# leggedrobotics/art_planner

Hardware: NVIDIA H100
Metric: pose-validity checks/s (higher is better)
Workload: dtype f32

## Files before the change

### art_planner_b200/csrc/artp_capi.cu

```cuda
#include <cassert>
#include <climits>
#include <cmath>
#include <cstdlib>
#include <cstring>
#include <cudaTypedefs.h>
#include <type_traits>
#include <vector>

#include "artp_internal.h"
#include "artp_kernels.cuh"
#include "artp_tiles.cuh"

namespace artp_api {

constexpr int kMaxSlices = 9;
constexpr int kMaxStoreSmem = 200 * 1024, kMaxTileSmem = 200 * 1024, kMaxGroupsSmem = 160 * 1024;

struct QueueCtr { uint32_t end, claim; };
struct alignas(32) BoxQueues { QueueCtr big, reach, group; };
struct Counters { BoxQueues q; uint32_t defer; };

struct Shape { int grid = 0, block = 0, smem = 0; };

struct Pipeline {
  enum { kBig, kReach, kGroup };
  Counters* d_ctr = nullptr;
  artp::BoxRec* recs[3] = {};
  uint32_t* d_defer = nullptr;
  size_t recs_cap = 0;
  BoxQueues* d_slices = nullptr;
  unsigned long long* d_compact_state = nullptr;
  size_t compact_state_cap = 0;
  uint32_t compact_epoch = 0;
  artp::TileCfg tile_cfg[2] = {};
  CUtensorMap tile_map[2][2];
  Shape tile[2];
  Shape groups;
  Shape grouping;
  int tcap = 0;
  int tcap_override = 0;
  int mode = 0;
  uint8_t* h_small_out = nullptr;
  bool deferred_unread = false;
  cudaStream_t streams[4] = {};
  cudaStream_t& copy_stream = streams[0];
  cudaStream_t& box_stream = streams[1];
  cudaStream_t& group_stream = streams[2];
  cudaStream_t& tile_stream = streams[3];
  cudaEvent_t order_ev[2 * kMaxSlices + 3] = {};
  cudaEvent_t *const copy_ev = order_ev, *const slice_ev = order_ev + kMaxSlices;
  cudaEvent_t& box_ev = order_ev[2 * kMaxSlices];
  cudaEvent_t &group_ev = order_ev[2 * kMaxSlices + 1], &tile_ev = order_ev[2 * kMaxSlices + 2];
  int timing = 0;
  cudaEvent_t ev[6] = {};
  bool ev_valid = false;
  ~Pipeline() {
    for (cudaStream_t s : streams) if (s) { cudaStreamSynchronize(s); cudaStreamDestroy(s); }
    for (cudaEvent_t e : order_ev) if (e) cudaEventDestroy(e);
    for (cudaEvent_t e : ev) if (e) cudaEventDestroy(e);
    for (artp::BoxRec* r : recs) cudaFree(r);
    cudaFree(d_ctr); cudaFree(d_defer); cudaFree(d_slices); cudaFree(d_compact_state);
    if (h_small_out) cudaFreeHost(h_small_out);
  }
};

}

using namespace artp_api;

namespace {

thread_local std::string g_create_error;

__global__ void reverse_columns_kernel(const float* __restrict__ layer, float* __restrict__ H, int nx, int nz, int pitch) {
  const size_t total = (size_t)pitch * nz;
  for (size_t i = blockIdx.x * (size_t)blockDim.x + threadIdx.x; i < total; i += (size_t)gridDim.x * blockDim.x) {
    const int z = (int)(i / pitch), x = (int)(i - (size_t)z * pitch);
    H[i] = (x < nx) ? layer[x + (size_t)(nz - 1 - z) * nx] * 1.0f + 0.0f : 0.0f;
  }
}

__global__ void build_level_kernel(const float* __restrict__ H, const float2* __restrict__ prevT,
                                   const unsigned char* __restrict__ prevNF, const unsigned char* __restrict__ mergeable,
                                   float2* __restrict__ T, unsigned char* __restrict__ NF, int nx, int nz, int pitch, int half) {
  const size_t total = (size_t)pitch * nz;
  for (size_t i = blockIdx.x * (size_t)blockDim.x + threadIdx.x; i < total; i += (size_t)gridDim.x * blockDim.x) {
    const int z = (int)(i / pitch), x = (int)(i - (size_t)z * pitch);
    if (x >= nx) { T[i] = make_float2(0.f, 0.f); NF[i] = 0; continue; }
    const int x2 = min(x + half, nx - 1), z2 = min(z + half, nz - 1);
    const size_t id[4] = {(size_t)z * pitch + x, (size_t)z * pitch + x2, (size_t)z2 * pitch + x, (size_t)z2 * pitch + x2};
    float mx = -CUDART_INF_F, mn = CUDART_INF_F;
    unsigned char nf = 0;
#pragma unroll
    for (int q = 0; q < 4; ++q) {
      if (prevT) {
        const float2 v = prevT[id[q]];
        mx = fmaxf(mx, v.x); mn = fminf(mn, v.y); nf |= prevNF[id[q]];
      } else {
        const float h = H[id[q]];
        mx = fmaxf(mx, h);
        if (fabsf(h) < CUDART_INF_F) mn = fminf(mn, h); else nf |= 1;
        nf |= mergeable[id[q]];
      }
    }
    T[i] = make_float2(mx, mn);
    NF[i] = nf;
  }
}

__global__ void build_codes_kernel(const float2* __restrict__ T, const unsigned char* __restrict__ NF, uint32_t* __restrict__ C,
                                   size_t n, float base, float step) {
  const float top = artp::code_dec(base, step, artp::kCodeMax);
  for (size_t i = blockIdx.x * (size_t)blockDim.x + threadIdx.x; i < n; i += (size_t)gridDim.x * blockDim.x) {
    const float2 v = T[i];
    uint32_t cM = 0, cm = artp::kCodeNone;
    if (v.x > top) cM = artp::kCodeNone;
    else if (v.x > -CUDART_INF_F) {
      uint32_t lo = 1, hi = artp::kCodeMax;
      while (lo < hi) {
        const uint32_t mid = (lo + hi) >> 1;
        if (artp::code_dec(base, step, mid) >= v.x) hi = mid; else lo = mid + 1;
      }
      cM = lo;
    }
    if (v.y <= top) {
      uint32_t lo = 0, hi = artp::kCodeMax;
      while (lo < hi) {
        const uint32_t mid = (lo + hi + 1) >> 1;
        if (artp::code_dec(base, step, mid) <= v.y) lo = mid; else hi = mid - 1;
      }
      cm = lo;
    }
    C[i] = artp::code_word(cM, cm, NF[i] & 3u);
  }
}

void code_scale_of(float lo, float hi, float& base, float& step) {
  base = lo <= hi ? lo : 0.0f;
  int e = -126;
  while (e < 127 && artp::code_dec(base, std::ldexp(1.0f, e), artp::kCodeMax) < hi) ++e;
  step = std::ldexp(1.0f, e);
}
void code_scale(const float* layer, size_t n, float& base, float& step) {
  float lo = HUGE_VALF, hi = -HUGE_VALF;
  for (size_t i = 0; i < n; ++i) {
    const float v = layer[i] * 1.0f + 0.0f;
    if (std::fabs(v) < HUGE_VALF) { lo = std::min(lo, v); hi = std::max(hi, v); }
  }
  code_scale_of(lo, hi, base, step);
}

struct PlaneSlot { unsigned long long key; uint32_t lo, hi; };
constexpr unsigned long long kEmptyKey = ~0ull;
__device__ __forceinline__ unsigned long long plane_key(int kx, int kz, int kd) {
  return ((unsigned long long)(uint32_t)(kx & 0xffff) << 48) | ((unsigned long long)(uint32_t)(kz & 0xffff) << 32) | (uint32_t)kd;
}
__device__ __forceinline__ uint32_t plane_slot_hash(unsigned long long k) {
  k ^= k >> 33; k *= 0xff51afd7ed558ccdull; k ^= k >> 33; k *= 0xc4ceb9fe1a85ec53ull; k ^= k >> 33;
  return (uint32_t)k;
}
__global__ void plane_table_clear_kernel(PlaneSlot* tab, size_t cap) {
  for (size_t i = blockIdx.x * (size_t)blockDim.x + threadIdx.x; i < cap; i += (size_t)gridDim.x * blockDim.x) {
    tab[i].key = kEmptyKey; tab[i].lo = 0xffffffffu; tab[i].hi = 0u;
  }
}
__device__ __forceinline__ bool cell_tri_plane(const artp::Field& f, int x, int x_off, int z, int u, float pl[4]) {
  float hA, hB, hC, hD;
  artp::load_cell(f, x, z, hA, hB, hC, hD);
  const bool ok = u == 0 ? (artp::finitef(hA) && artp::finitef(hB) && artp::finitef(hC))
// ... 363 lines not shown
int check_states(Handle* h, const T* d_states, size_t n, uint8_t* d_valid, cudaStream_t s, const HostFeed* feed = nullptr) {
  artp::Work w;
  if constexpr (std::is_same_v<T, float>) w.s2f = d_states; else w.s2 = d_states;
  w.valid = d_valid;
  w.n_items = (uint32_t)n;
  return run_items(h, w, s, feed);
}

template <typename T>
int check_poses(Handle* h, const T* states, size_t n, uint8_t* valid, bool on_device, cudaStream_t stream) {
  TRY(check_common(h, n));
  if (n == 0) return ARTP_OK;
  if (!states || !valid) return null_buffer(h);
  if (on_device) {
    CU_TRY(h, cudaSetDevice(h->device));
    ChainScope cs(h, 0, stream);
    if (cs.rc) return cs.rc;
    return check_states(h, states, n, valid, stream);
  }
  if (n <= (size_t)artp::kSmallBatch && !h->pipe->timing) {
    artp::SmallBatch sb;
    for (size_t i = 0; i < n * 7; ++i) (&sb.s[0][0])[i] = (double)states[i];
    return check_poses_small(h, sb, n, valid);
  }
  char* r[2];
  TRY(host_call_begin(h, {n * 7 * sizeof(T), n}, r));
  const HostFeed feed = std::is_same_v<T, float>
                            ? HostFeed{(const char*)states, r[0], 7 * sizeof(T), 256 * 1024, {0.08f, 0.17f, 0.25f, 0.25f, 0.25f}}
                            : HostFeed{(const char*)states, r[0], 7 * sizeof(T), 128 * 1024, {0.06f, 0.14f, 0.20f, 0.20f, 0.20f, 0.20f}};
  TRY(check_states(h, (const T*)r[0], n, (uint8_t*)r[1], h->stream, &feed));
  CU_TRY(h, cudaMemcpyAsync(valid, r[1], n, cudaMemcpyDeviceToHost, h->stream));
  return host_call_end(h, true);
}

int motion_items(Handle* h, size_t n, int n_steps) {
  if (n_steps < 0) { h->err = "n_steps < 0"; return ARTP_E_INVALID; }
  return check_common(h, n * ((size_t)n_steps + 1));
}
int check_motions_on(Handle* h, const double* d_s1, const double* d_s2, size_t n, int n_steps, uint8_t* d_valid, cudaStream_t s) {
  TRY(launch(h, fill_u8_kernel, grid_for(h, n, 256, 8), 256, 0, s, d_valid, n, 1));
  const size_t items = n * ((size_t)n_steps + 1);
  artp::Work w;
  w.s1 = d_s1; w.s2 = d_s2; w.valid = d_valid; w.n_items = (uint32_t)items; w.steps = n_steps; w.edge_mode = 1;
  return run_items(h, w, s);
}

__global__ void edge_prefix_kernel(const uint8_t* __restrict__ item_valid, const uint32_t* __restrict__ item_off, size_t n,
                                   int32_t* __restrict__ valid_prefix) {
  for (size_t e = blockIdx.x * (size_t)blockDim.x + threadIdx.x; e < n; e += (size_t)gridDim.x * blockDim.x) {
    const uint32_t o0 = item_off[e];
    valid_prefix[e] = (int32_t)artp::leading_valid(item_valid + o0, item_off[e + 1] - o0);
  }
}

int check_items_prefix(Handle* h, const double* d_s1, const double* d_s2, size_t n, const uint32_t* d_item_off,
                       size_t total_items, uint8_t* d_item_valid, int32_t* d_valid_prefix, void* stream, int quotient) {
  TRY(check_common(h, total_items));
  if (n == 0) return ARTP_OK;
  if (!d_s1 || !d_s2 || !d_item_off || !d_valid_prefix || (total_items && !d_item_valid)) {
    return null_buffer(h);
  }
  if (n >= 0xFFFFFFFFull) { h->err = "too many edges"; return ARTP_E_INVALID; }
  CU_TRY(h, cudaSetDevice(h->device));
  cudaStream_t s = (cudaStream_t)stream;
  ChainScope cs(h, 0, s);
  if (cs.rc) return cs.rc;
  if (total_items) {
    artp::Work w;
    w.s1 = d_s1; w.s2 = d_s2; w.valid = d_item_valid; w.n_items = (uint32_t)total_items;
    w.item_off = d_item_off; w.n_edges = (uint32_t)n; w.quotient = quotient;
    TRY(run_items(h, w, s));
  }
  return launch(h, edge_prefix_kernel, grid_for(h, n, 256, 8), 256, 0, s, d_item_valid, d_item_off, n, d_valid_prefix);
}

int check_items_prefix_host(Handle* h, const double* s1, const double* s2, const std::vector<uint32_t>& off, int quotient,
                            int32_t* valid_prefix) {
  const size_t n = off.size() - 1, total = off[n], sb = n * 7 * sizeof(double);
  char* r[5];
  TRY(host_call_begin(h, {sb, sb, (n + 1) * sizeof(uint32_t), n * sizeof(int32_t), total}, r));
  CU_TRY(h, cudaMemcpyAsync(r[0], s1, sb, cudaMemcpyHostToDevice, h->stream));
  CU_TRY(h, cudaMemcpyAsync(r[1], s2, sb, cudaMemcpyHostToDevice, h->stream));
  CU_TRY(h, cudaMemcpyAsync(r[2], off.data(), (n + 1) * sizeof(uint32_t), cudaMemcpyHostToDevice, h->stream));
  TRY(check_items_prefix(h, (const double*)r[0], (const double*)r[1], n, (const uint32_t*)r[2], total, (uint8_t*)r[4],
                         (int32_t*)r[3], h->stream, quotient));
  CU_TRY(h, cudaMemcpyAsync(valid_prefix, r[3], n * sizeof(int32_t), cudaMemcpyDeviceToHost, h->stream));
  return host_call_end(h, true);
}

int pack_valid_bits(Handle* h, const uint8_t* d_valid, size_t n, uint32_t* d_bits, cudaStream_t s) {
  if (n == 0) return ARTP_OK;
  if (!d_valid || !d_bits) return null_buffer(h);
  CU_TRY(h, cudaSetDevice(h->device));
  const size_t words = (n + 31) / 32;
  return launch(h, pack_bits_kernel, grid_for(h, words * 32, 256, 8), 256, 0, s, d_valid, n, d_bits);
}

int timed_round_ms(Handle* h, float* ms, std::initializer_list<std::pair<int, int>> pairs) {
  const Pipeline& p = *h->pipe;
  if (!ms) return ARTP_E_INVALID;
  if (!p.timing || !p.ev_valid) { h->err = "timing not enabled or no call recorded"; return ARTP_E_INVALID; }
  CU_TRY(h, cudaSetDevice(h->device));
  CU_TRY(h, cudaEventSynchronize(p.ev[5]));
  for (const auto& [from, to] : pairs) CU_TRY(h, cudaEventElapsedTime(ms++, p.ev[from], p.ev[to]));
  return ARTP_OK;
}

template <typename... P>
int fit_shape(Handle* h, void (*kernel)(P...), int block, int smem, Shape& out) {
  int per_sm = 0;
  CU_TRY(h, cudaOccupancyMaxActiveBlocksPerMultiprocessor(&per_sm, kernel, block, smem));
  out = {h->sm_count * std::max(per_sm, 1), block, smem};
  return ARTP_OK;
}

int set_shapes(Handle* h, const int span[2][2], int tcap, int store) {
  Pipeline& p = *h->pipe;
  TRY(fit_shape(h, artp::box_items_block_kernel, artp::kBlockStageThreads, store, p.grouping));
  p.tcap = tcap;
  PFN_cuTensorMapEncodeTiled encode = nullptr;
  cudaDriverEntryPointQueryResult qres;
  if (cudaGetDriverEntryPoint("cuTensorMapEncodeTiled", (void**)&encode, cudaEnableDefault, &qres) != cudaSuccess || !encode) {
    h->err = "cuTensorMapEncodeTiled not available from the driver"; return ARTP_E_CUDA;
  }
  h->chk.reach_tw = 0; h->chk.reach_th = 0;
  for (int q = 0; q < 2; ++q) {
    const int tw = std::min((span[q][0] + 3 + 3 + 3) & ~3, 256), th = std::min(span[q][1] + 3, 256);
    artp::TileCfg tc;
    tc.tw = tw; tc.th = th; tc.bytes = (uint32_t)tw * th * 4; tc.stride = (tc.bytes + 127u) & ~127u;
    tc.slots = (tc.stride > 2048) ? 1 : 2;
    int wpc = 8;
    while (wpc > 1 && (size_t)wpc * tc.slots * tc.stride + 128 > 72 * 1024) wpc >>= 1;
    if ((size_t)wpc * tc.slots * tc.stride + 128 > kMaxTileSmem) {
      if (q == 1) { p.tile[1] = Shape{}; continue; }
      tc.tw = 64; tc.th = 64; tc.bytes = 64 * 64 * 4; tc.stride = tc.bytes; tc.slots = 1; wpc = 4;
    }
    const cuuint64_t gdim[2] = {(cuuint64_t)h->pitch, (cuuint64_t)h->cols};
    const cuuint64_t gstr[1] = {(cuuint64_t)h->pitch * sizeof(float)};
    const cuuint32_t box[2] = {(cuuint32_t)tc.tw, (cuuint32_t)tc.th};
    const cuuint32_t one[2] = {1, 1};
    for (int layer = 0; layer < 2; ++layer) {
      const CUresult cr = encode(&p.tile_map[q][layer], CU_TENSOR_MAP_DATA_TYPE_FLOAT32, 2, h->d_H[layer], gdim, gstr, box, one,
                                 CU_TENSOR_MAP_INTERLEAVE_NONE, CU_TENSOR_MAP_SWIZZLE_NONE, CU_TENSOR_MAP_L2_PROMOTION_L2_128B,
                                 CU_TENSOR_MAP_FLOAT_OOB_FILL_NONE);
      if (cr != CUDA_SUCCESS) { h->err = "cuTensorMapEncodeTiled failed (" + std::to_string((int)cr) + ")"; return ARTP_E_CUDA; }
    }
    tc.x_off = h->win_row0;
    p.tile_cfg[q] = tc;
    p.tile[q] = {0, wpc * 32, (int)((size_t)wpc * tc.slots * tc.stride + 128)};
    if (q == 1) { h->chk.reach_tw = tc.tw; h->chk.reach_th = tc.th; }
  }
  p.groups = Shape{};
  if (h->chk.reach_tw && p.tile_cfg[1].tw <= 127 && p.tile_cfg[1].th <= 255) {
    const int gsm = artp::kMaxTileWarps * 8 * (int)p.tile_cfg[1].stride + 128;
    if (gsm <= kMaxGroupsSmem && !std::getenv("ARTP_NO_GROUPS")) {
      TRY(fit_shape(h, artp::reach_groups_kernel, artp::kMaxTileWarps * 32, gsm, p.groups));
    }
  }
  for (Shape& t : p.tile)
    if (t.block) TRY(fit_shape(h, artp::box_tiles_warp_kernel, t.block, t.smem, t));
  return ARTP_OK;
}

}

int artp_api::take_sticky_error(Handle* h) {
  if (h->h_err && *(volatile uint32_t*)h->h_err) {
    const uint32_t e = *(volatile uint32_t*)h->h_err;
    *(volatile uint32_t*)h->h_err = 0;
    if (e & 2u) {
      h->err = "a box reached outside this handle's map window (artp_set_map_window: route samples to the shard that holds them, "
               "halo >= box half-diagonal + offsets); affected poses were marked invalid";
      return ARTP_E_WINDOW;
    }
    h->err = "plane-grouping stage overflow: a zone exceeded its shared-memory store; affected poses were marked invalid";
    return ARTP_E_LIMIT;
  }
  return ARTP_OK;
}

int artp_api::check_states_f32(Handle* h, const float* d_states, size_t n, uint8_t* d_valid, cudaStream_t s) {
  return check_states(h, d_states, n, d_valid, s);
}

int artp_api::check_states_cta(Handle* h, const double* d_states, const uint32_t* d_count, const uint32_t* d_stop, size_t max_n,
                               uint8_t* d_valid, cudaStream_t s) {
  if (max_n == 0) return ARTP_OK;
  TRY(launch(h, artp::pose_states_kernel, (unsigned)max_n, 256, h->pipe->grouping.smem, s, h->chk, d_states, d_count, d_stop,
             d_valid, h->pipe->tcap, h->d_err));
  h->pipe->ev_valid = false;
  return ARTP_OK;
}

int artp_api::compact_valid(Handle* h, const uint8_t* d_valid, size_t n, int64_t base, void* d_indices, uint32_t* d_count,
                            cudaStream_t s, bool bits, bool u32) {
  Pipeline& p = *h->pipe;
  if (n == 0) { CU_TRY(h, cudaMemsetAsync(d_count, 0, sizeof(uint32_t), s)); return ARTP_OK; }
  ChainScope cs(h, 1, s);
  if (cs.rc) return cs.rc;
  const size_t nt = (n + kCompactTile - 1) / kCompactTile;
  if (p.compact_state_cap < nt + 1 || p.compact_epoch + 1 >= kCompactEpochs) {
    TRY(grow(h, p.d_compact_state, p.compact_state_cap, nt + 1));
    CU_TRY(h, cudaMemsetAsync(p.d_compact_state, 0, p.compact_state_cap * sizeof(unsigned long long), s));
    p.compact_epoch = 0;
  }
  const uint32_t epoch = ++p.compact_epoch;
  auto run = [&](auto kernel, auto* indices) {
    return launch(h, kernel, (unsigned)nt, kCompactThreads, 0, s, d_valid, n, base, p.d_compact_state, epoch, indices, d_count);
  };
  if (bits) return run(compact_kernel<true, int64_t>, (int64_t*)d_indices);
  if (u32) return run(compact_kernel<false, uint32_t>, (uint32_t*)d_indices);
  return run(compact_kernel<false, int64_t>, (int64_t*)d_indices);
}

extern "C" {

const char* artp_version(void) { return "artp 0.1 sm_90a"; }

const char* artp_last_error(const artp_handle* hh) {
  if (!hh) return g_create_error.c_str();
  return reinterpret_cast<const Handle*>(hh)->err.c_str();
}

int artp_create(const artp_params* params, artp_handle** out) {
  if (!params || !out) { g_create_error = "null argument"; return ARTP_E_INVALID; }
  *out = nullptr;
  int ndev = 0;
  cudaError_t e = cudaGetDeviceCount(&ndev);
  if (e != cudaSuccess || ndev == 0) {
    g_create_error = std::string("no CUDA device: ") + cudaGetErrorString(e);
    return ARTP_E_CUDA;
  }
  if (params->device < 0 || params->device >= ndev) { g_create_error = "bad device ordinal"; return ARTP_E_INVALID; }
  if (!(params->torso_length > 0 && params->torso_width > 0 && params->torso_height > 0 && params->reach_x > 0 &&
        params->reach_y > 0 && params->reach_z > 0)) {
    g_create_error = "box dimensions must be positive";
    return ARTP_E_INVALID;
  }
  Handle* h = new Handle();
  h->p = *params;
  h->device = params->device;
  auto fail = [&](const char* what, cudaError_t ce) {
    g_create_error = std::string(what) + ": " + cudaGetErrorString(ce);
    artp_destroy(reinterpret_cast<artp_handle*>(h));
    return ARTP_E_CUDA;
  };
  if ((e = cudaSetDevice(h->device)) != cudaSuccess) return fail("cudaSetDevice", e);
  cudaDeviceProp prop;
  if ((e = cudaGetDeviceProperties(&prop, h->device)) != cudaSuccess) return fail("cudaGetDeviceProperties", e);
  h->sm_count = prop.multiProcessorCount;
  cudaFuncAttributes fa;
  if ((e = cudaFuncGetAttributes(&fa, artp::box_tiles_warp_kernel)) != cudaSuccess)
    return fail("no usable kernel image (built for sm_90a)", e);
  int prio_least = 0, prio_greatest = 0;
  if ((e = cudaDeviceGetStreamPriorityRange(&prio_least, &prio_greatest)) != cudaSuccess) return fail("cudaDeviceGetStreamPriorityRange", e);
  if ((e = cudaStreamCreateWithFlags(&h->stream, cudaStreamNonBlocking)) != cudaSuccess) return fail("cudaStreamCreate", e);
  Pipeline& p = *(h->pipe = new Pipeline());
  for (cudaStream_t& st : p.streams) {
    e = &st == &p.tile_stream ? cudaStreamCreateWithPriority(&st, cudaStreamNonBlocking, prio_greatest)
                              : cudaStreamCreateWithFlags(&st, cudaStreamNonBlocking);
    if (e != cudaSuccess) return fail("cudaStreamCreate", e);
  }
  for (cudaEvent_t& ev : p.order_ev)
    if ((e = cudaEventCreateWithFlags(&ev, cudaEventDisableTiming)) != cudaSuccess) return fail("cudaEventCreate", e);
  for (cudaEvent_t& ev : h->chain_ev)
    if ((e = cudaEventCreateWithFlags(&ev, cudaEventDisableTiming)) != cudaSuccess) return fail("cudaEventCreate", e);
  if ((e = cudaMalloc(&p.d_slices, kMaxSlices * sizeof(BoxQueues))) != cudaSuccess) return fail("cudaMalloc", e);
  if ((e = cudaMalloc(&p.d_ctr, sizeof(Counters))) != cudaSuccess) return fail("cudaMalloc", e);
  if ((e = cudaHostAlloc((void**)&p.h_small_out, 64, cudaHostAllocMapped)) != cudaSuccess) return fail("cudaHostAlloc", e);
  const std::pair<const void*, int> smem_caps[] = {
      {(const void*)artp::pose_small_kernel, kMaxStoreSmem}, {(const void*)artp::pose_states_kernel, kMaxStoreSmem},
      {(const void*)artp::box_items_block_kernel, kMaxStoreSmem}, {(const void*)artp::box_tiles_warp_kernel, kMaxTileSmem},
      {(const void*)artp::reach_groups_kernel, kMaxGroupsSmem}};
  for (const auto& [k, bytes] : smem_caps)
    if ((e = cudaFuncSetAttribute(k, cudaFuncAttributeMaxDynamicSharedMemorySize, bytes)) != cudaSuccess)
      return fail("cudaFuncSetAttribute", e);
  if ((e = cudaHostAlloc((void**)&h->h_err, 64, cudaHostAllocMapped)) != cudaSuccess) return fail("cudaHostAlloc", e);
  *h->h_err = 0;
  if ((e = cudaHostGetDevicePointer((void**)&h->d_err, h->h_err, 0)) != cudaSuccess) return fail("cudaHostGetDevicePointer", e);
  h->cnn = artp_cnn::create(h->device, h->sm_count);
  artp::Checker& c = h->chk;
  std::memset(&c, 0, sizeof(c));
  c.side[0][0] = (float)params->torso_length; c.side[0][1] = (float)params->torso_width; c.side[0][2] = (float)params->torso_height;
  c.side[1][0] = (float)params->reach_x; c.side[1][1] = (float)params->reach_y; c.side[1][2] = (float)params->reach_z;
  c.torso_off[0] = (float)params->torso_off_x; c.torso_off[1] = (float)params->torso_off_y;
  c.torso_off[2] = (float)(params->torso_off_z - params->feet_off_z);
  c.feet_ox = (float)params->feet_off_x; c.feet_oy = (float)params->feet_off_y;
  c.unknown_untraversable = params->unknown_space_untraversable ? 1 : 0;
  *out = reinterpret_cast<artp_handle*>(h);
  return ARTP_OK;
}

void artp_destroy(artp_handle* hh) {
  if (!hh) return;
  Handle* h = reinterpret_cast<Handle*>(hh);
  cudaSetDevice(h->device);
  if (h->stream) { cudaStreamSynchronize(h->stream); cudaStreamDestroy(h->stream); }
  delete h->pipe;
  for (int k = 0; k < 2; ++k) for (int l = 0; l <= artp::kMaxLevel; ++l) { cudaFree(h->d_T[k][l]); cudaFree(h->d_C[k][l]); }
  cudaFree(h->d_H[0]); cudaFree(h->d_H[1]); cudaFree(h->d_stage); cudaFree(h->d_simplify);
  sampling_free(h);
  roadmap_free(h);
  planner_free(h);
  if (h->h_err) cudaFreeHost(h->h_err);
  for (cudaEvent_t ev : h->chain_ev) if (ev) cudaEventDestroy(ev);
  artp_cnn::destroy(h->cnn);
  delete h;
// ... 378 lines not shown
```

### art_planner_b200/csrc/artp_tiles.cuh

```cuda
#pragma once

#include <cuda.h>

#include "artp_kernels.cuh"

namespace artp {

constexpr uint32_t kDeferReachBit = 0x80000000u;
constexpr int kTileChunk = 8;

__device__ __forceinline__ uint32_t smem_addr(const void* p) { return (uint32_t)__cvta_generic_to_shared(p); }
__device__ __forceinline__ void mbar_init(uint64_t* bar, uint32_t count) {
  asm volatile("mbarrier.init.shared::cta.b64 [%0], %1;" ::"r"(smem_addr(bar)), "r"(count));
}
__device__ __forceinline__ void mbar_expect_tx(uint64_t* bar, uint32_t bytes) {
  asm volatile("mbarrier.arrive.expect_tx.shared::cta.b64 _, [%0], %1;" ::"r"(smem_addr(bar)), "r"(bytes) : "memory");
}
__device__ __forceinline__ void mbar_wait(uint64_t* bar, uint32_t parity) {
  asm volatile(
      "{\n\t"
      ".reg .pred P1;\n\t"
      "TWAIT_LOOP:\n\t"
      "mbarrier.try_wait.parity.shared::cta.b64 P1, [%0], %1;\n\t"
      "@P1 bra TWAIT_DONE;\n\t"
      "bra TWAIT_LOOP;\n\t"
      "TWAIT_DONE:\n\t"
      "}" ::"r"(smem_addr(bar)), "r"(parity) : "memory");
}
__device__ __forceinline__ void tma_tile_2d(void* dst, const CUtensorMap* map, uint64_t* bar, int c0, int c1) {
  asm volatile(
      "cp.async.bulk.tensor.2d.shared::cluster.global.mbarrier::complete_tx::bytes [%0], [%1, {%3, %4}], [%2];" ::"r"(
          smem_addr(dst)),
      "l"(map), "r"(smem_addr(bar)), "r"(c0), "r"(c1)
      : "memory");
}

constexpr int kMaxTileWarps = 8;

__device__ __forceinline__ unsigned char* warp_tile_slots(unsigned char* smem, const TileCfg& tc, int n, uint64_t bars[2]) {
  const int wid = threadIdx.x >> 5;
  unsigned char* slots = reinterpret_cast<unsigned char*>((reinterpret_cast<uintptr_t>(smem) + 127) & ~(uintptr_t)127) +
                         (size_t)wid * n * tc.stride;
  if ((threadIdx.x & 31) == 0) { mbar_init(&bars[0], 1); mbar_init(&bars[1], 1); }
  asm volatile("fence.mbarrier_init.release.cluster;" ::: "memory");
  __syncwarp();
  return slots;
}

__global__ void __launch_bounds__(kMaxTileWarps * 32, 3)
box_tiles_warp_kernel(const Checker c, const __grid_constant__ CUtensorMap map0, const __grid_constant__ CUtensorMap map1,
                      const TileCfg tc, const Work w, const BoxRec* __restrict__ recs, const uint32_t* __restrict__ rec_count,
                      uint32_t* __restrict__ work_counter, uint32_t* __restrict__ defer_count, uint32_t* __restrict__ defer_list,
                      uint32_t queue_bit, int force_defer) {
  extern __shared__ __align__(128) unsigned char tile_smem[];
  __shared__ WarpScratch ws_all[kMaxTileWarps];
  __shared__ uint64_t bars[kMaxTileWarps][2];
  const int lane = threadIdx.x & 31, wid = threadIdx.x >> 5;
  WarpScratch& ws = ws_all[wid];
  unsigned char* slots = warp_tile_slots(tile_smem, tc, tc.slots, bars[wid]);
  uint32_t phase[2] = {0u, 0u};
  const uint32_t total = *rec_count;
  auto prefetch = [&](uint32_t ri, int slot) {
    const int x0 = rec_x0(recs + ri), z0 = rec_z0(recs + ri);
    const uint32_t fl = rec_flags(recs + ri);
    if (lane == 0) {
      mbar_expect_tx(&bars[wid][slot], tc.bytes);
      tma_tile_2d(slots + (size_t)slot * tc.stride, (fl & 7u) ? &map1 : &map0, &bars[wid][slot], (x0 & ~3) - tc.x_off, z0);
    }
  };
  const uint32_t nwarps2 = 2u * gridDim.x * (blockDim.x >> 5);
  uint32_t next_r0 = 0, next_n = 0;
  const uint32_t first_seen = *(volatile const uint32_t*)work_counter;
  const bool fixed_claims = total - min(first_seen, total) >= (nwarps2 >> 2) * (uint32_t)kTileChunk;
  auto claim = [&]() {
    if (lane == 0) {
      next_n = (uint32_t)kTileChunk;
      if (!fixed_claims) {
        const uint32_t cur = *(volatile const uint32_t*)work_counter;
        next_n = cur < total ? min(max((total - cur) / nwarps2, 1u), (uint32_t)kTileChunk) : 1u;
      }
      next_r0 = atomicAdd(work_counter, next_n);
    }
  };
  if (!fixed_claims) claim();
  for (;;) {
    if (fixed_claims) claim();
    const uint32_t r0 = __shfl_sync(kFull, next_r0, 0), nclaim = __shfl_sync(kFull, next_n, 0);
    if (r0 >= total) break;
    if (!fixed_claims) claim();
    const uint32_t r1 = min(r0 + nclaim, total);
    if (force_defer) {
      if (lane == 0) for (uint32_t ri = r0; ri < r1; ++ri) defer_list[atomicAdd(defer_count, 1u)] = ri | queue_bit;
      continue;
    }
    for (uint32_t ri = r0; ri < r1; ++ri) {
      const int slot = (int)(ri - r0) & (tc.slots - 1);
      if (tc.slots == 1 || ri == r0) { __syncwarp(); prefetch(ri, slot); }
      const BoxRec r = load_rec(recs + ri);
      if (tc.slots == 2 && ri + 1 < r1) { __syncwarp(); prefetch(ri + 1, slot ^ 1); }
      const uint32_t slot_item = r.item;
      const bool foot = (r.flags & 7) != 0;
      int dead = 0;
      if (lane == 0) dead = (*(volatile const uint8_t*)(w.valid + slot_item) == 0);
      dead = __shfl_sync(kFull, dead, 0);
      mbar_wait(&bars[wid][slot], phase[slot]);
      phase[slot] ^= 1u;
      if (dead) continue;
      BoxCtx b;
      rec_to_ctx(c, r, b);
      int res;
      if ((b.x1 - b.x0) + 4 > tc.tw || (b.z1 - b.z0) + 1 > tc.th) {
        res = R_DEFER;
      } else {
        const ZoneView zv{reinterpret_cast<const float*>(slots + (size_t)slot * tc.stride) + (b.x0 & 3), tc.tw};
        res = box_collide_warp<true>(foot ? c.f[1] : c.f[0], b, zv, ws, lane, c.cell_margin, (r.flags & REC_NEEDS_REDUCE) != 0,
                                     (r.flags & REC_ALLFINITE) != 0, (r.flags & REC_MERGEFREE) != 0);
      }
      if (lane == 0) {
        if (res == R_DEFER) defer_list[atomicAdd(defer_count, 1u)] = ri | queue_bit;
        else if (box_fails(foot, res)) w.valid[slot_item] = 0;
      }
    }
  }
}

constexpr int kGroupRounds = 8;
constexpr int kGroupTasks = 64;

__global__ void __launch_bounds__(kMaxTileWarps * 32, 3)
reach_groups_kernel(const Checker c, const __grid_constant__ CUtensorMap map1, const TileCfg tc, const Work w,
                    const BoxRec* __restrict__ recs, const uint32_t* __restrict__ rec_count, uint32_t* __restrict__ work_counter) {
  extern __shared__ __align__(128) unsigned char tile_smem[];
  __shared__ uint64_t bars[kMaxTileWarps][2];
  __shared__ uint16_t tasks_all[kMaxTileWarps][4][kGroupTasks];
  __shared__ __align__(16) float ctx_all[kMaxTileWarps][4][16];
  const int lane = threadIdx.x & 31, wid = threadIdx.x >> 5, g = lane >> 3, gl = lane & 7;
  const Field& f = c.f[1];
  unsigned char* slots = warp_tile_slots(tile_smem, tc, 8, bars[wid]);
  uint16_t* tasks = tasks_all[wid][g];
  uint32_t phase = 0u;
  const uint32_t total = *rec_count;
  const unsigned gshift = (unsigned)g * 8u;
  auto prefetch = [&](uint32_t first, int slot) {
    const uint32_t ri = first + (uint32_t)g;
    int x0 = 0, z0 = 0;
    const bool act = ri < total;
    if (act && gl == 0) { x0 = rec_x0(recs + ri); z0 = rec_z0(recs + ri); }
    const int nact = (int)min(4u, total - first);
    if (lane == 0) mbar_expect_tx(&bars[wid][slot], (uint32_t)nact * tc.bytes);
#pragma unroll 1
    for (int q = 0; q < nact; ++q) {
      const int sx = __shfl_sync(kFull, x0, q * 8), sz = __shfl_sync(kFull, z0, q * 8);
      if (lane == 0) tma_tile_2d(slots + (size_t)(slot * 4 + q) * tc.stride, &map1, &bars[wid][slot], (sx & ~3) - tc.x_off, sz);
    }
  };
  const uint32_t nwarps8 = 8u * gridDim.x * (blockDim.x >> 5);
  uint32_t next_r0 = 0, next_n = 0;
  auto claim = [&]() {
    if (lane == 0) {
      const uint32_t cur = *(volatile const uint32_t*)work_counter;
      next_n = 4u * (cur < total ? min(max((total - cur) / nwarps8, 1u), (uint32_t)kGroupRounds) : 1u);
      next_r0 = atomicAdd(work_counter, next_n);
    }
  };
  claim();
  for (;;) {
    const uint32_t r0 = __shfl_sync(kFull, next_r0, 0), nclaim = __shfl_sync(kFull, next_n, 0);
    if (r0 >= total) break;
    claim();
    const int nrounds = (int)((min(r0 + nclaim, total) - r0 + 3u) / 4u);
    __syncwarp();
    prefetch(r0, 0);
#pragma unroll 1
    for (int round = 0; round < nrounds; ++round) {
      const int slot = round & 1;
      const uint32_t ri = r0 + 4u * (uint32_t)round + (uint32_t)g;
      const bool act = ri < total;
      BoxRec r = {};
      if (act) r = load_rec(recs + ri);
      if (round + 1 < nrounds) { __syncwarp(); prefetch(r0 + 4u * (uint32_t)(round + 1), slot ^ 1); }
      int alive = 0;
      if (act && gl == 0) alive = (*(volatile const uint8_t*)(w.valid + r.item) != 0);
      alive = __shfl_sync(kFull, alive, 0, 8);
      mbar_wait(&bars[wid][slot], (phase >> slot) & 1u);
      phase ^= 1u << slot;
      __syncwarp();
      bool gdone = !(act && alive);
      BoxCtx b;
      rec_to_ctx(c, r, b);
      if (gdone) { b.x0 = b.z0 = 0; b.x1 = b.z1 = 1; }
      if (gl == 0) {
        float* cx = ctx_all[wid][g];
#pragma unroll
        for (int i = 0; i < 9; ++i) cx[i] = b.R1[i];
        cx[9] = b.P[0]; cx[10] = b.P[1]; cx[11] = b.P[2]; cx[12] = b.minB;
        cx[13] = __int_as_float(b.x0); cx[14] = __int_as_float(b.z0);
      }
      const float* tile = reinterpret_cast<const float*>(slots + (size_t)(slot * 4 + g) * tc.stride) + (b.x0 & 3);
      const float top = b.maxB + (1e-4f + 4e-6f * fabsf(b.maxB));
      bool ghit = false;
      const bool allFinite = (r.flags & REC_ALLFINITE) != 0;
      {
        const float xr = box_half_extent(b.R1, b.side, 0) + 1e-4f, zr = box_half_extent(b.R1, b.side, 2) + 1e-4f;
        const int vx0 = max(b.x0, (int)ceilf((b.P[0] - xr) * f.iW)), vx1 = min(b.x1, (int)floorf((b.P[0] + xr) * f.iW));
        const int vz0 = max(b.z0, (int)ceilf((b.P[2] - zr) * f.iD)), vz1 = min(b.z1, (int)floorf((b.P[2] + zr) * f.iD));
        const int nXi = max(vx1 - vx0 + 1, 0), nZi = max(vz1 - vz0 + 1, 0), nVi = nXi * nZi;
        const float* tin = tile + (vz0 - b.z0) * tc.tw + (vx0 - b.x0);
        int maxNV = gdone ? 0 : nVi;
        maxNV = __reduce_max_sync(kFull, maxNV);
        const uint32_t magicX = magic_for(nXi);
#pragma unroll 1
        for (int t0 = 0; t0 < maxNV; t0 += 8) {
          const int t = t0 + gl;
          bool hit = false;
          if (!gdone && t < nVi) {
            const int zi = (nXi > 1) ? (int)__umulhi((uint32_t)t, magicX) : t, xi = t - zi * nXi;
            const float h = tin[zi * tc.tw + xi];
            hit = h > b.minB && h < top && vertex_inside(b, (vx0 + xi) * f.sW, h, (vz0 + zi) * f.sD);
            if (hit && !allFinite)
              hit = vertex_in_kept_triangle<true>(ZoneView{tile, tc.tw}, b.x1 - b.x0 + 1, b.z1 - b.z0 + 1, vx0 - b.x0 + xi,
                                                  vz0 - b.z0 + zi, b.minB);
          }
          if ((__ballot_sync(kFull, hit) >> gshift) & 0xffu) { ghit = true; gdone = true; }
          if (__all_sync(kFull, gdone)) break;
        }
      }
      __syncwarp();
      int nt = 0;
      {
        float pc[3];
        box_corner(b, gl, pc);
        const float gx = pc[0] * f.iW, gz = pc[2] * f.iD;
        const int cxl = (int)floorf(gx - c.cell_margin), cxh = (int)floorf(gx + c.cell_margin);
        const int czl = (int)floorf(gz - c.cell_margin), czh = (int)floorf(gz + c.cell_margin);
        const int oxl = __shfl_xor_sync(kFull, cxl, 4), oxh = __shfl_xor_sync(kFull, cxh, 4);
        const int ozl = __shfl_xor_sync(kFull, czl, 4), ozh = __shfl_xor_sync(kFull, czh, 4);
        const bool same = (oxl == cxl) & (oxh == cxh) & (ozl == czl) & (ozh == czh);
        const bool mine = !gdone && !((gl & 4) && same);
        bool ok[4];
#pragma unroll
        for (int sub = 0; sub < 4; ++sub) {
          const int ccx = (sub & 1) ? cxh : cxl, ccz = (sub & 2) ? czh : czl;
          ok[sub] = mine && !((sub & 1) && cxh == cxl) && !((sub & 2) && czh == czl) && ccx >= b.x0 && ccx < b.x1 && ccz >= b.z0 &&
                    ccz < b.z1;
        }
        int base = 0;
#pragma unroll
        for (int sub = 0; sub < 4; ++sub) {
          const unsigned gm = (__ballot_sync(kFull, ok[sub]) >> gshift) & 0xffu;
          if (ok[sub]) {
            const int slot_i = base + __popc(gm & ((1u << gl) - 1u));
            const int ccx = (sub & 1) ? cxh : cxl, ccz = (sub & 2) ? czh : czl;
            const int code = (((ccx - b.x0) << 8) | (ccz - b.z0)) << 1;
            tasks[2 * slot_i] = (uint16_t)code; tasks[2 * slot_i + 1] = (uint16_t)(code | 1);
          }
          base += __popc(gm);
        }
        nt = 2 * base;
      }
      __syncwarp();
      {
        const int n0 = __shfl_sync(kFull, nt, 0), n1 = __shfl_sync(kFull, nt, 8), n2 = __shfl_sync(kFull, nt, 16), n3 = __shfl_sync(kFull, nt, 24);
        const int o1 = n0, o2 = n0 + n1, o3 = o2 + n2, NT = o3 + n3;
        unsigned hit_groups = 0u;
#pragma unroll 1
        for (int j0 = 0; j0 < NT; j0 += 32) {
          const int j = j0 + lane;
          if (j < NT) {
            const int gi = (j >= o1) + (j >= o2) + (j >= o3);
            const int q = j - (gi == 0 ? 0 : gi == 1 ? o1 : gi == 2 ? o2 : o3);
            const int tk = tasks_all[wid][gi][q];
            const float4* cx = reinterpret_cast<const float4*>(ctx_all[wid][gi]);
            const float4 c0 = cx[0], c1 = cx[1], c2 = cx[2], c3 = cx[3];
            BoxCtx tb;
            tb.R1[0] = c0.x; tb.R1[1] = c0.y; tb.R1[2] = c0.z; tb.R1[3] = c0.w; tb.R1[4] = c1.x; tb.R1[5] = c1.y; tb.R1[6] = c1.z;
            tb.R1[7] = c1.w; tb.R1[8] = c2.x; tb.P[0] = c2.y; tb.P[1] = c2.z; tb.P[2] = c2.w; tb.minB = c3.x;
            tb.side[0] = c.side[1][0]; tb.side[1] = c.side[1][1]; tb.side[2] = c.side[1][2];
            const int tx0 = __float_as_int(c3.y), tz0 = __float_as_int(c3.z);
            const bool isUp = (tk & 1) == 0;
            const int lx = tk >> 9, lz = (tk >> 1) & 0xff, ccx = tx0 + lx, ccz = tz0 + lz;
            const float* p = reinterpret_cast<const float*>(slots + (size_t)(slot * 4 + gi) * tc.stride) + (tx0 & 3) + lz * tc.tw + lx;
            const float hA = p[0], hB = p[1], hC = p[tc.tw], hD = p[tc.tw + 1];
            if (tri_kept(isUp, hA, hB, hC, hD, tb.minB)) {
              float pl[4], cxs[4], czs[4];
              cell_plane(f, isUp, ccx, ccz, hA, hB, hC, hD, pl);
              const int nc = box_plane(tb, pl, 4, cxs, czs);
              const int tcx = isUp ? ccx : ccx + 1, tcz = isUp ? ccz : ccz + 1;
              bool hit = false;
#pragma unroll
              for (int i = 0; i < 4; ++i) hit = hit || (i < nc && on_tri(f, isUp, tcx, tcz, cxs[i], czs[i]));
              if (hit) hit_groups |= 1u << gi;
            }
          }
        }
        __syncwarp();
        hit_groups = __reduce_or_sync(kFull, hit_groups);
        if ((hit_groups >> g) & 1u) ghit = true;
      }
      if (gl == 0 && act && alive && box_fails(true, ghit ? R_HIT : R_FREE)) w.valid[r.item] = 0;
      __syncwarp();
    }
  }
}

}
```

Before: 2.068 billion.

## Compact surviving reach boxes into a ring before the plane stage

Splits the reach-groups kernel into two phases. Boxes that survive the vertex stage are appended to a per-warp ring of up to 8 contexts, and the plane-test stage runs only once four live boxes have accumulated, so warp lanes are not wasted on groups that already finished. Tile slots move from fixed double-buffered pairs to an 11-slot pool tracked by a free bitmask, and the shared-memory cap is raised to fit them. The cost is more shared memory per block, which may reduce occupancy, plus extra bookkeeping. There is also a risk of slot exhaustion or ordering bugs, because the ring holds tiles across rounds.

```diff
diff --git a/art_planner_b200/csrc/artp_capi.cu b/art_planner_b200/csrc/artp_capi.cu
--- a/art_planner_b200/csrc/artp_capi.cu
+++ b/art_planner_b200/csrc/artp_capi.cu
@@ -14,7 +14,7 @@
 namespace artp_api {
 
 constexpr int kMaxSlices = 9;
-constexpr int kMaxStoreSmem = 200 * 1024, kMaxTileSmem = 200 * 1024, kMaxGroupsSmem = 160 * 1024;
+constexpr int kMaxStoreSmem = 200 * 1024, kMaxTileSmem = 200 * 1024, kMaxGroupsSmem = 216 * 1024;
 
 struct QueueCtr { uint32_t end, claim; };
 struct alignas(32) BoxQueues { QueueCtr big, reach, group; };
@@ -684,7 +684,7 @@
   }
   p.groups = Shape{};
   if (h->chk.reach_tw && p.tile_cfg[1].tw <= 127 && p.tile_cfg[1].th <= 255) {
-    const int gsm = artp::kMaxTileWarps * 8 * (int)p.tile_cfg[1].stride + 128;
+    const int gsm = artp::kMaxTileWarps * artp::kGroupSlots * (int)p.tile_cfg[1].stride + 128;
     if (gsm <= kMaxGroupsSmem && !std::getenv("ARTP_NO_GROUPS")) {
       TRY(fit_shape(h, artp::reach_groups_kernel, artp::kMaxTileWarps * 32, gsm, p.groups));
     }
diff --git a/art_planner_b200/csrc/artp_tiles.cuh b/art_planner_b200/csrc/artp_tiles.cuh
--- a/art_planner_b200/csrc/artp_tiles.cuh
+++ b/art_planner_b200/csrc/artp_tiles.cuh
@@ -126,6 +126,8 @@
 
 constexpr int kGroupRounds = 8;
 constexpr int kGroupTasks = 64;
+constexpr int kGroupSlots = 11;
+constexpr int kGroupRing = 8;
 
 __global__ void __launch_bounds__(kMaxTileWarps * 32, 3)
 reach_groups_kernel(const Checker c, const __grid_constant__ CUtensorMap map1, const TileCfg tc, const Work w,
@@ -133,26 +135,34 @@
   extern __shared__ __align__(128) unsigned char tile_smem[];
   __shared__ uint64_t bars[kMaxTileWarps][2];
   __shared__ uint16_t tasks_all[kMaxTileWarps][4][kGroupTasks];
-  __shared__ __align__(16) float ctx_all[kMaxTileWarps][4][16];
+  __shared__ __align__(16) float ring_ctx[kMaxTileWarps][kGroupRing][16];
+  __shared__ uint32_t ring_item[kMaxTileWarps][kGroupRing];
+  __shared__ uint8_t ring_slot[kMaxTileWarps][kGroupRing];
   const int lane = threadIdx.x & 31, wid = threadIdx.x >> 5, g = lane >> 3, gl = lane & 7;
   const Field& f = c.f[1];
-  unsigned char* slots = warp_tile_slots(tile_smem, tc, 8, bars[wid]);
+  unsigned char* slots = warp_tile_slots(tile_smem, tc, kGroupSlots, bars[wid]);
   uint16_t* tasks = tasks_all[wid][g];
   uint32_t phase = 0u;
+  uint32_t free_slots = (1u << kGroupSlots) - 1u;
+  int head = 0, nring = 0;
   const uint32_t total = *rec_count;
   const unsigned gshift = (unsigned)g * 8u;
-  auto prefetch = [&](uint32_t first, int slot) {
+  auto prefetch = [&](uint32_t first, int bar) {
     const uint32_t ri = first + (uint32_t)g;
     int x0 = 0, z0 = 0;
-    const bool act = ri < total;
-    if (act && gl == 0) { x0 = rec_x0(recs + ri); z0 = rec_z0(recs + ri); }
+    if (ri < total && gl == 0) { x0 = rec_x0(recs + ri); z0 = rec_z0(recs + ri); }
     const int nact = (int)min(4u, total - first);
-    if (lane == 0) mbar_expect_tx(&bars[wid][slot], (uint32_t)nact * tc.bytes);
+    if (lane == 0) mbar_expect_tx(&bars[wid][bar], (uint32_t)nact * tc.bytes);
+    int mine = 0;
 #pragma unroll 1
     for (int q = 0; q < nact; ++q) {
+      const int s = __ffs(free_slots) - 1;
+      free_slots &= free_slots - 1u;
+      if (g == q) mine = s;
       const int sx = __shfl_sync(kFull, x0, q * 8), sz = __shfl_sync(kFull, z0, q * 8);
-      if (lane == 0) tma_tile_2d(slots + (size_t)(slot * 4 + q) * tc.stride, &map1, &bars[wid][slot], (sx & ~3) - tc.x_off, sz);
-    }
+      if (lane == 0) tma_tile_2d(slots + (size_t)s * tc.stride, &map1, &bars[wid][bar], (sx & ~3) - tc.x_off, sz);
+    }
+    return mine;
   };
   const uint32_t nwarps8 = 8u * gridDim.x * (blockDim.x >> 5);
   uint32_t next_r0 = 0, next_n = 0;
@@ -164,41 +174,40 @@
     }
   };
   claim();
+  uint32_t r0 = 0;
+  int round = 0, nrounds = 0, next_slot = 0;
+  bool more = true;
   for (;;) {
-    const uint32_t r0 = __shfl_sync(kFull, next_r0, 0), nclaim = __shfl_sync(kFull, next_n, 0);
-    if (r0 >= total) break;
-    claim();
-    const int nrounds = (int)((min(r0 + nclaim, total) - r0 + 3u) / 4u);
-    __syncwarp();
-    prefetch(r0, 0);
-#pragma unroll 1
-    for (int round = 0; round < nrounds; ++round) {
-      const int slot = round & 1;
+    if (round == nrounds && more) {
+      r0 = __shfl_sync(kFull, next_r0, 0);
+      const uint32_t nclaim = __shfl_sync(kFull, next_n, 0);
+      more = r0 < total;
+      if (more) {
+        claim();
+        nrounds = (int)((min(r0 + nclaim, total) - r0 + 3u) / 4u);
+        round = 0;
+        __syncwarp();
+        next_slot = prefetch(r0, 0);
+      }
+    }
+    if (round < nrounds) {
+      const int bar = round & 1, slot = next_slot;
       const uint32_t ri = r0 + 4u * (uint32_t)round + (uint32_t)g;
       const bool act = ri < total;
       BoxRec r = {};
       if (act) r = load_rec(recs + ri);
-      if (round + 1 < nrounds) { __syncwarp(); prefetch(r0 + 4u * (uint32_t)(round + 1), slot ^ 1); }
+      if (round + 1 < nrounds) { __syncwarp(); next_slot = prefetch(r0 + 4u * (uint32_t)(round + 1), bar ^ 1); }
       int alive = 0;
       if (act && gl == 0) alive = (*(volatile const uint8_t*)(w.valid + r.item) != 0);
       alive = __shfl_sync(kFull, alive, 0, 8);
-      mbar_wait(&bars[wid][slot], (phase >> slot) & 1u);
-      phase ^= 1u << slot;
+      mbar_wait(&bars[wid][bar], (phase >> bar) & 1u);
+      phase ^= 1u << bar;
       __syncwarp();
       bool gdone = !(act && alive);
       BoxCtx b;
       rec_to_ctx(c, r, b);
-      if (gdone) { b.x0 = b.z0 = 0; b.x1 = b.z1 = 1; }
-      if (gl == 0) {
-        float* cx = ctx_all[wid][g];
-#pragma unroll
-        for (int i = 0; i < 9; ++i) cx[i] = b.R1[i];
-        cx[9] = b.P[0]; cx[10] = b.P[1]; cx[11] = b.P[2]; cx[12] = b.minB;
-        cx[13] = __int_as_float(b.x0); cx[14] = __int_as_float(b.z0);
-      }
-      const float* tile = reinterpret_cast<const float*>(slots + (size_t)(slot * 4 + g) * tc.stride) + (b.x0 & 3);
+      const float* tile = reinterpret_cast<const float*>(slots + (size_t)slot * tc.stride) + (b.x0 & 3);
       const float top = b.maxB + (1e-4f + 4e-6f * fabsf(b.maxB));
-      bool ghit = false;
       const bool allFinite = (r.flags & REC_ALLFINITE) != 0;
       {
         const float xr = box_half_extent(b.R1, b.side, 0) + 1e-4f, zr = box_half_extent(b.R1, b.side, 2) + 1e-4f;
@@ -221,85 +230,125 @@
               hit = vertex_in_kept_triangle<true>(ZoneView{tile, tc.tw}, b.x1 - b.x0 + 1, b.z1 - b.z0 + 1, vx0 - b.x0 + xi,
                                                   vz0 - b.z0 + zi, b.minB);
           }
-          if ((__ballot_sync(kFull, hit) >> gshift) & 0xffu) { ghit = true; gdone = true; }
+          if ((__ballot_sync(kFull, hit) >> gshift) & 0xffu) gdone = true;
           if (__all_sync(kFull, gdone)) break;
         }
       }
-      __syncwarp();
-      int nt = 0;
-      {
-        float pc[3];
-        box_corner(b, gl, pc);
-        const float gx = pc[0] * f.iW, gz = pc[2] * f.iD;
-        const int cxl = (int)floorf(gx - c.cell_margin), cxh = (int)floorf(gx + c.cell_margin);
-        const int czl = (int)floorf(gz - c.cell_margin), czh = (int)floorf(gz + c.cell_margin);
-        const int oxl = __shfl_xor_sync(kFull, cxl, 4), oxh = __shfl_xor_sync(kFull, cxh, 4);
-        const int ozl = __shfl_xor_sync(kFull, czl, 4), ozh = __shfl_xor_sync(kFull, czh, 4);
-        const bool same = (oxl == cxl) & (oxh == cxh) & (ozl == czl) & (ozh == czh);
-        const bool mine = !gdone && !((gl & 4) && same);
-        bool ok[4];
+      const unsigned surv = __ballot_sync(kFull, !gdone && gl == 0);
+      if (!gdone && gl == 0) {
+        const int e = (head + nring + __popc(surv & ((1u << lane) - 1u))) & (kGroupRing - 1);
+        float4* cx = reinterpret_cast<float4*>(ring_ctx[wid][e]);
+        cx[0] = make_float4(b.R1[0], b.R1[1], b.R1[2], b.R1[3]);
+        cx[1] = make_float4(b.R1[4], b.R1[5], b.R1[6], b.R1[7]);
+        cx[2] = make_float4(b.R1[8], b.P[0], b.P[1], b.P[2]);
+        cx[3] = make_float4(b.minB, __int_as_float(b.x0), __int_as_float(b.z0), __int_as_float((b.x1 - b.x0) | ((b.z1 - b.z0) << 16)));
+        ring_item[wid][e] = r.item;
+        ring_slot[wid][e] = (uint8_t)slot;
+      }
+      free_slots |= __reduce_or_sync(kFull, (act && gdone && gl == 0) ? 1u << slot : 0u);
+      nring += __popc(surv);
+      ++round;
+    }
+    if (nring < 4 && (more || nring == 0)) {
+      if (!more) break;
+      continue;
+    }
+    __syncwarp();
+    const int nf = min(nring, 4);
+    const int e = (head + g) & (kGroupRing - 1);
+    int alive = 0;
+    uint32_t item = 0;
+    if (g < nf && gl == 0) {
+      item = ring_item[wid][e];
+      alive = (*(volatile const uint8_t*)(w.valid + item) != 0);
+    }
+    const bool live = __shfl_sync(kFull, alive, 0, 8) != 0;
+    const int slot = ring_slot[wid][e];
+    int nt = 0;
+    {
+      BoxCtx b;
+      const float4* cx = reinterpret_cast<const float4*>(ring_ctx[wid][e]);
+      const float4 c0 = cx[0], c1 = cx[1], c2 = cx[2], c3 = cx[3];
+      b.R1[0] = c0.x; b.R1[1] = c0.y; b.R1[2] = c0.z; b.R1[3] = c0.w; b.R1[4] = c1.x; b.R1[5] = c1.y; b.R1[6] = c1.z;
+      b.R1[7] = c1.w; b.R1[8] = c2.x; b.P[0] = c2.y; b.P[1] = c2.z; b.P[2] = c2.w;
+      b.side[0] = c.side[1][0]; b.side[1] = c.side[1][1]; b.side[2] = c.side[1][2];
+      b.x0 = __float_as_int(c3.y); b.z0 = __float_as_int(c3.z);
+      const int ext = __float_as_int(c3.w);
+      b.x1 = b.x0 + (ext & 0xffff); b.z1 = b.z0 + (ext >> 16);
+      float pc[3];
+      box_corner(b, gl, pc);
+      const float gx = pc[0] * f.iW, gz = pc[2] * f.iD;
+      const int cxl = (int)floorf(gx - c.cell_margin), cxh = (int)floorf(gx + c.cell_margin);
+      const int czl = (int)floorf(gz - c.cell_margin), czh = (int)floorf(gz + c.cell_margin);
+      const int oxl = __shfl_xor_sync(kFull, cxl, 4), oxh = __shfl_xor_sync(kFull, cxh, 4);
+      const int ozl = __shfl_xor_sync(kFull, czl, 4), ozh = __shfl_xor_sync(kFull, czh, 4);
+      const bool same = (oxl == cxl) & (oxh == cxh) & (ozl == czl) & (ozh == czh);
+      const bool mine = live && !((gl & 4) && same);
+      bool ok[4];
 #pragma unroll
-        for (int sub = 0; sub < 4; ++sub) {
+      for (int sub = 0; sub < 4; ++sub) {
+        const int ccx = (sub & 1) ? cxh : cxl, ccz = (sub & 2) ? czh : czl;
+        ok[sub] = mine && !((sub & 1) && cxh == cxl) && !((sub & 2) && czh == czl) && ccx >= b.x0 && ccx < b.x1 && ccz >= b.z0 &&
+                  ccz < b.z1;
+      }
+      int base = 0;
+#pragma unroll
+      for (int sub = 0; sub < 4; ++sub) {
+        const unsigned gm = (__ballot_sync(kFull, ok[sub]) >> gshift) & 0xffu;
+        if (ok[sub]) {
+          const int slot_i = base + __popc(gm & ((1u << gl) - 1u));
           const int ccx = (sub & 1) ? cxh : cxl, ccz = (sub & 2) ? czh : czl;
-          ok[sub] = mine && !((sub & 1) && cxh == cxl) && !((sub & 2) && czh == czl) && ccx >= b.x0 && ccx < b.x1 && ccz >= b.z0 &&
-                    ccz < b.z1;
+          const int code = (((ccx - b.x0) << 8) | (ccz - b.z0)) << 1;
+          tasks[2 * slot_i] = (uint16_t)code; tasks[2 * slot_i + 1] = (uint16_t)(code | 1);
         }
-        int base = 0;
+        base += __popc(gm);
+      }
+      nt = 2 * base;
+    }
+    __syncwarp();
+    {
+      const int n0 = __shfl_sync(kFull, nt, 0), n1 = __shfl_sync(kFull, nt, 8), n2 = __shfl_sync(kFull, nt, 16), n3 = __shfl_sync(kFull, nt, 24);
+      const int o1 = n0, o2 = n0 + n1, o3 = o2 + n2, NT = o3 + n3;
+      unsigned hit_groups = 0u;
+#pragma unroll 1
+      for (int j0 = 0; j0 < NT; j0 += 32) {
+        const int j = j0 + lane;
+        if (j < NT) {
+          const int gi = (j >= o1) + (j >= o2) + (j >= o3);
+          const int q = j - (gi == 0 ? 0 : gi == 1 ? o1 : gi == 2 ? o2 : o3);
+          const int tk = tasks_all[wid][gi][q];
+          const int ge = (head + gi) & (kGroupRing - 1);
+          const float4* cx = reinterpret_cast<const float4*>(ring_ctx[wid][ge]);
+          const float4 c0 = cx[0], c1 = cx[1], c2 = cx[2], c3 = cx[3];
+          BoxCtx tb;
+          tb.R1[0] = c0.x; tb.R1[1] = c0.y; tb.R1[2] = c0.z; tb.R1[3] = c0.w; tb.R1[4] = c1.x; tb.R1[5] = c1.y; tb.R1[6] = c1.z;
+          tb.R1[7] = c1.w; tb.R1[8] = c2.x; tb.P[0] = c2.y; tb.P[1] = c2.z; tb.P[2] = c2.w; tb.minB = c3.x;
+          tb.side[0] = c.side[1][0]; tb.side[1] = c.side[1][1]; tb.side[2] = c.side[1][2];
+          const int tx0 = __float_as_int(c3.y), tz0 = __float_as_int(c3.z);
+          const bool isUp = (tk & 1) == 0;
+          const int lx = tk >> 9, lz = (tk >> 1) & 0xff, ccx = tx0 + lx, ccz = tz0 + lz;
+          const float* p = reinterpret_cast<const float*>(slots + (size_t)ring_slot[wid][ge] * tc.stride) + (tx0 & 3) + lz * tc.tw + lx;
+          const float hA = p[0], hB = p[1], hC = p[tc.tw], hD = p[tc.tw + 1];
+          if (tri_kept(isUp, hA, hB, hC, hD, tb.minB)) {
+            float pl[4], cxs[4], czs[4];
+            cell_plane(f, isUp, ccx, ccz, hA, hB, hC, hD, pl);
+            const int nc = box_plane(tb, pl, 4, cxs, czs);
+            const int tcx = isUp ? ccx : ccx + 1, tcz = isUp ? ccz : ccz + 1;
+            bool hit = false;
 #pragma unroll
-        for (int sub = 0; sub < 4; ++sub) {
-          const unsigned gm = (__ballot_sync(kFull, ok[sub]) >> gshift) & 0xffu;
-          if (ok[sub]) {
-            const int slot_i = base + __popc(gm & ((1u << gl) - 1u));
-            const int ccx = (sub & 1) ? cxh : cxl, ccz = (sub & 2) ? czh : czl;
-            const int code = (((ccx - b.x0) << 8) | (ccz - b.z0)) << 1;
-            tasks[2 * slot_i] = (uint16_t)code; tasks[2 * slot_i + 1] = (uint16_t)(code | 1);
-          }
-          base += __popc(gm);
-        }
-        nt = 2 * base;
-      }
-      __syncwarp();
-      {
-        const int n0 = __shfl_sync(kFull, nt, 0), n1 = __shfl_sync(kFull, nt, 8), n2 = __shfl_sync(kFull, nt, 16), n3 = __shfl_sync(kFull, nt, 24);
-        const int o1 = n0, o2 = n0 + n1, o3 = o2 + n2, NT = o3 + n3;
-        unsigned hit_groups = 0u;
-#pragma unroll 1
-        for (int j0 = 0; j0 < NT; j0 += 32) {
-          const int j = j0 + lane;
-          if (j < NT) {
-            const int gi = (j >= o1) + (j >= o2) + (j >= o3);
-            const int q = j - (gi == 0 ? 0 : gi == 1 ? o1 : gi == 2 ? o2 : o3);
-            const int tk = tasks_all[wid][gi][q];
-            const float4* cx = reinterpret_cast<const float4*>(ctx_all[wid][gi]);
-            const float4 c0 = cx[0], c1 = cx[1], c2 = cx[2], c3 = cx[3];
-            BoxCtx tb;
-            tb.R1[0] = c0.x; tb.R1[1] = c0.y; tb.R1[2] = c0.z; tb.R1[3] = c0.w; tb.R1[4] = c1.x; tb.R1[5] = c1.y; tb.R1[6] = c1.z;
-            tb.R1[7] = c1.w; tb.R1[8] = c2.x; tb.P[0] = c2.y; tb.P[1] = c2.z; tb.P[2] = c2.w; tb.minB = c3.x;
-            tb.side[0] = c.side[1][0]; tb.side[1] = c.side[1][1]; tb.side[2] = c.side[1][2];
-            const int tx0 = __float_as_int(c3.y), tz0 = __float_as_int(c3.z);
-            const bool isUp = (tk & 1) == 0;
-            const int lx = tk >> 9, lz = (tk >> 1) & 0xff, ccx = tx0 + lx, ccz = tz0 + lz;
-            const float* p = reinterpret_cast<const float*>(slots + (size_t)(slot * 4 + gi) * tc.stride) + (tx0 & 3) + lz * tc.tw + lx;
-            const float hA = p[0], hB = p[1], hC = p[tc.tw], hD = p[tc.tw + 1];
-            if (tri_kept(isUp, hA, hB, hC, hD, tb.minB)) {
-              float pl[4], cxs[4], czs[4];
-              cell_plane(f, isUp, ccx, ccz, hA, hB, hC, hD, pl);
-              const int nc = box_plane(tb, pl, 4, cxs, czs);
-              const int tcx = isUp ? ccx : ccx + 1, tcz = isUp ? ccz : ccz + 1;
-              bool hit = false;
-#pragma unroll
-              for (int i = 0; i < 4; ++i) hit = hit || (i < nc && on_tri(f, isUp, tcx, tcz, cxs[i], czs[i]));
-              if (hit) hit_groups |= 1u << gi;
-            }
+            for (int i = 0; i < 4; ++i) hit = hit || (i < nc && on_tri(f, isUp, tcx, tcz, cxs[i], czs[i]));
+            if (hit) hit_groups |= 1u << gi;
           }
         }
-        __syncwarp();
-        hit_groups = __reduce_or_sync(kFull, hit_groups);
-        if ((hit_groups >> g) & 1u) ghit = true;
-      }
-      if (gl == 0 && act && alive && box_fails(true, ghit ? R_HIT : R_FREE)) w.valid[r.item] = 0;
+      }
       __syncwarp();
-    }
+      hit_groups = __reduce_or_sync(kFull, hit_groups);
+      if (gl == 0 && live && box_fails(true, ((hit_groups >> g) & 1u) ? R_HIT : R_FREE)) w.valid[item] = 0;
+    }
+    free_slots |= __reduce_or_sync(kFull, (g < nf && gl == 0) ? 1u << slot : 0u);
+    head = (head + nf) & (kGroupRing - 1);
+    nring -= nf;
+    __syncwarp();
   }
 }
 
diff --git a/profiles/reach_round_mix.py b/profiles/reach_round_mix.py
--- /dev/null
+++ b/profiles/reach_round_mix.py
@@ -0,0 +1,117 @@
+import argparse
+import json
+import math
+import os
+import sys
+
+ROOT = os.path.dirname(os.path.dirname(os.path.abspath(__file__)))
+sys.path.insert(0, ROOT)
+
+import numpy as np
+
+import bench
+from art_planner_b200 import synth
+from oracle.orc import Oracle
+
+ST_VERTEX, ST_PLANE, ST_FREE, ST_OUTSIDE = 5, 6, 7, 255
+
+STAGE_SASS = {"round": 265, "v_fixed": 96, "v_body": 132, "collect": 177, "t_fixed": 24, "t_body": 376}
+TWO_PHASE_SASS = {"append": 54, "flush": 53}
+
+
+def inner_vertices(zv):
+    s = np.sqrt(zv.astype(np.float64))
+    return np.maximum(np.round(s) - 2, 1) ** 2
+
+
+def model(st, hit, zv, tasks):
+    reach_st, reach_hit = st[:, 1:], hit[:, 1:]
+    early = reach_st < ST_VERTEX
+    invalid = ((early & (reach_hit == 0)) | (reach_st == ST_OUTSIDE)).any(axis=1)
+    inner = inner_vertices(zv[:, 1:])
+    items, ks = np.nonzero((reach_st >= ST_VERTEX) & (reach_st <= ST_FREE) & ~invalid[:, None])
+    rec_st = reach_st[items, ks]
+    rec_nv = inner[items, ks]
+    n = len(items)
+    S = STAGE_SASS
+    rounds = (n + 3) // 4
+    live_v, live_c, trips, own_trips, iters_before = [], [], [], [], []
+    failed = set()
+    survivors = 0
+    before = after = 0.0
+    for r in range(rounds):
+        sl = slice(4 * r, min(4 * r + 4, n))
+        it, es, nv = items[sl], rec_st[sl], rec_nv[sl]
+        alive = np.array([i not in failed for i in it])
+        lv = int(alive.sum())
+        open_ = alive & (es != ST_VERTEX)
+        lc = int(open_.sum())
+        t = int(math.ceil(nv[alive].max() / 8)) if lv else 0
+        own = [math.ceil(v / 8) for v in nv[alive]]
+        ti = math.ceil(lc * tasks / 32)
+        live_v.append(lv); live_c.append(lc); trips.append(t); own_trips.append(float(np.mean(own)) if own else 0.0)
+        iters_before.append(ti)
+        v = S["v_fixed"] + S["v_body"] * t
+        before += S["round"] + v + S["collect"] + S["t_fixed"] + S["t_body"] * ti
+        after += S["round"] + v + TWO_PHASE_SASS["append"]
+        survivors += lc
+        for i, e in zip(it, es):
+            if e == ST_FREE:
+                failed.add(int(i))
+    flushes = (survivors + 3) // 4
+    full, rest = divmod(survivors, 4)
+    iters_after = full * math.ceil(4 * tasks / 32) + (math.ceil(rest * tasks / 32) if rest else 0)
+    plane_after = flushes * (TWO_PHASE_SASS["flush"] + S["collect"] + S["t_fixed"]) + S["t_body"] * iters_after
+    after += plane_after
+    lc = np.array(live_c)
+    plane_before = sum(S["collect"] + S["t_fixed"] + S["t_body"] * i for i in iters_before)
+    dead_round_plane = sum(S["collect"] + S["t_fixed"] + S["t_body"] * i for i, c in zip(iters_before, live_c) if c < 4)
+    hist = lambda a: {str(k): int((np.asarray(a) == k).sum()) for k in range(5)}
+    return {
+        "records": n, "rounds": rounds,
+        "exit_share": {"vertex": round(float((rec_st == ST_VERTEX).mean()), 4), "plane_hit": round(float((rec_st == ST_PLANE).mean()), 4),
+                       "fall_through": round(float((rec_st == ST_FREE).mean()), 4)},
+        "live_at_vertex_stage": hist(live_v), "live_at_collection": hist(live_c),
+        "mean_live_at_collection": round(float(lc.mean()), 3),
+        "vertex_trips_mean": round(float(np.mean(trips)), 3), "own_trips_mean": round(float(np.mean(own_trips)), 3),
+        "task_iters_per_round_mean": round(float(np.mean(iters_before)), 3),
+        "plane_stage_runs": {"before": rounds, "after": flushes},
+        "task_iters_total": {"before": int(sum(iters_before)), "after": int(iters_after)},
+        "warp_instr_per_box": {"before": round(before / n, 1), "after": round(after / n, 1),
+                               "plane_before": round(plane_before / n, 1), "plane_after": round(plane_after / n, 1)},
+        "share_of_instr_in_plane_stages_of_rounds_with_dead_groups": round(dead_round_plane / before, 4),
+        "modelled_saving": round(1 - after / before, 4),
+    }
+
+
+def main():
+    p = argparse.ArgumentParser()
+    p.add_argument("--n", type=int, default=40_000, help="bench poses (a prefix of configs[1]'s)")
+    p.add_argument("--tasks", type=float, default=12.0, help="candidate tasks per open box (assumption, not measured)")
+    p.add_argument("--gpu", action="store_true", help="also read the real B' queue length on the GPU")
+    p.add_argument("--out", default=None, help="directory for reach_round_mix.json")
+    a = p.parse_args()
+    m, poses = bench.make_inputs(0, a.n)
+    o = Oracle(synth.PARAMS_YAML, "port")
+    o.set_map(m)
+    st, hit, zv = o.pose_box_stats(poses)
+    res = {"poses": a.n, "tasks_per_open_box": a.tasks, "model": model(st, hit, zv, a.tasks)}
+    if a.gpu:
+        import torch
+        import art_planner_b200 as ap
+        chk = ap.StateValidityChecker(synth.PARAMS_YAML, device=0)
+        chk.setMap(m)
+        chk.updateHeightField()
+        chk.isValidBatch(torch.from_numpy(poses).cuda())
+        torch.cuda.synchronize()
+        res["gpu_queue_records"] = int(chk.stats()["last_reach_plane_stage"])
+    line = json.dumps(res)
+    print(line)
+    if a.out:
+        os.makedirs(a.out, exist_ok=True)
+        with open(os.path.join(a.out, "reach_round_mix.json"), "w") as f:
+            f.write(line + "\n")
+
+
+if __name__ == "__main__":
+    main()
```

Result: no change. 2.076 billion (median of 6 runs) (+0.4%).
